# Acly/dlimgedit

Measured on AMD Instinct MI355X. Metric: images/sec encode+mask @1024x1024, higher is better.
Workload: dtype f16; 1 GPU; SAM vit_b encoder + 1 point prompt, 1 image(s)/GPU/step, 1024x1024 RGBA, inputs and masks resident in HBM; timed through the extension entry point dlimg_amd_encode_and_mask (device pointers in and out) -- the drop-in table itself, host buffers in and out, is `abi_path`; weights=seeded synthetic, lanes_per_gpu=4, lanes_fed_by_the_step_queue=3, requests_coalesced_per_pass=4, passes_queued_per_lane=2

## Files before the change

### dlimgedit_amd/csrc/kernels/decoder.hip

```cpp
#include "device_common.hpp"
#include "kernels.hpp"

#include <cstring>
#include <mutex>
#include <type_traits>

namespace dlimg {
namespace {

#include "gemm_f16_tile.inc"

constexpr int OUT_TOK = 5;
constexpr int DIM = 256;
constexpr int INNER = 128;
constexpr int HEADS = 8;
constexpr int NTOK_IMG = 4096;

template <int TOK, typename Prompts>
DLIMG_DEVICE void prompt_token_column(const Prompts& pr, int p, int c, const float* __restrict__ gauss,
                                      const float* __restrict__ point_embed, const float* __restrict__ not_a_point,
                                      const float* __restrict__ iou_token, const float* __restrict__ mask_tokens,
                                      float (&out)[TOK]) {
    constexpr int NPTS = TOK - OUT_TOK;
    out[0] = iou_token[c];
// ... 493 lines not shown
}

template <int TOK>
constexpr size_t TML_LDS = (size_t)(INNER * DIM + TL_ROW_SLICE<TOK> * INNER + TL_ROW_SLICE<TOK> * DIM) * 4 + 2 * TL_ROW_SLICE<TOK> * 8;
template <int TOK, int NR, int COLS>
DLIMG_DEVICE void token_merge_linear_body(const float* __restrict__ part, const k::TokenLinear& out,
                                          const float* __restrict__ out_wt, const k::TokenLinear& next, int p0, float* lds) {
    float* wt = lds;
    float* att = wt + INNER * DIM;
    float* y = att + TL_ROW_SLICE<TOK> * INNER;
    float2_t* stat_res = reinterpret_cast<float2_t*>(y + TL_ROW_SLICE<TOK> * DIM);
    float2_t* stat_in = stat_res + TL_ROW_SLICE<TOK>;
    const int row0 = p0 * TOK, row1 = row0 + NR;
    const int first = blockIdx.x * COLS;
    const int c = threadIdx.x, lane = lane_id(), wave = c >> 6;
    for (int k = wave; k < INNER; k += 4) glds16(out_wt + (size_t)k * DIM + lane * 4, wt + k * DIM);
    TokenColumn col = token_column_prefetch(next, first, row0, row1);
    float res[NR];
#pragma unroll
    for (int r = 0; r < NR; ++r) res[r] = out.resid.x ? out.resid.x[(size_t)(row0 + r) * DIM + c] : 0.f;
    const bool res_ln = out.resid.x && out.resid.ln_w;
    const float rw = res_ln ? out.resid.ln_w[c] : 1.f, rb = res_ln ? out.resid.ln_b[c] : 0.f;
    const float ob = out.b ? out.b[c] : 0.f;
    const float nw = next.in.ln_w ? next.in.ln_w[c] : 1.f, nb = next.in.ln_w ? next.in.ln_b[c] : 0.f;
    float nadd[NR];
#pragma unroll
    for (int r = 0; r < NR; ++r) nadd[r] = next.in.add ? next.in.add[(size_t)(row0 + r) * DIM + c] : 0.f;
    merge_partials<TOK, NR>(part, p0, 0, att);
    if (res_ln) token_row_stats(out.resid, row1, stat_res - row0, row0);
    asm volatile("s_waitcnt vmcnt(0)" ::: "memory");
    __syncthreads();
    float acc[NR];
#pragma unroll
    for (int r = 0; r < NR; ++r) acc[r] = 0.f;
#pragma unroll 2
    for (int k4 = 0; k4 < INNER / 4; ++k4) {
        float w[4];
        float4_t a[NR];
#pragma unroll
        for (int i = 0; i < 4; ++i) w[i] = wt[(4 * k4 + i) * DIM + c];
#pragma unroll
        for (int r = 0; r < NR; ++r) a[r] = reinterpret_cast<const float4_t*>(att)[r * (INNER / 4) + k4];
#pragma unroll
        for (int r = 0; r < NR; ++r)
#pragma unroll
            for (int i = 0; i < 4; ++i) acc[r] = fmaf(a[r][i], w[i], acc[r]);
    }
#pragma unroll
    for (int r = 0; r < NR; ++r) {
        float v = acc[r] + ob;
        if (out.resid.x) v += res_ln ? (res[r] - stat_res[r][0]) * stat_res[r][1] * rw + rb : res[r];
        y[r * DIM + c] = v;
        if (blockIdx.x == 0) out.Y[(size_t)(row0 + r) * DIM + c] = v;
    }
    __syncthreads();
    if (next.in.ln_w) {
        lds_row_stats(y, NR, next.in.eps, stat_in);
        __syncthreads();
    }
    if (next.in.ln_w || next.in.add) {
#pragma unroll
        for (int r = 0; r < NR; ++r) {
            float v = y[r * DIM + c];
            if (next.in.ln_w) v = (v - stat_in[r][0]) * stat_in[r][1] * nw + nb;
            y[r * DIM + c] = v + nadd[r];
        }
        __syncthreads();
    }
#pragma unroll 1
    for (int i = 0; i < COLS / 4; ++i) {
        const TokenColumn following = token_column_prefetch(next, first + 4 * min(i + 1, COLS / 4 - 1), row0, row1);
        token_linear_columns<TOK, NR>(next, first + 4 * i, y, nullptr, nullptr, col, row0);
        col = following;
    }
}
template <int TOK, int COLS>
__global__ __launch_bounds__(256) void token_merge_linear_kernel(const float* __restrict__ part, k::TokenLinear out,
                                                                 const float* __restrict__ out_wt, k::TokenLinear next, int P) {
    extern __shared__ __attribute__((aligned(16))) float lds[];
    token_merge_linear_body<TOK, TOK, COLS>(part, out, out_wt, next, blockIdx.y, lds);
}

constexpr int HEAD_THREADS = 1024;
static_assert(DIM == 64 * 4, "one float4 of the weight row per lane");

template <int N_OUT>
DLIMG_DEVICE void head_layer(const float* x , const float* __restrict__ w, const float* __restrict__ b, int n_out,
                             bool relu, float* y) {
    constexpr int WAVES = HEAD_THREADS / 64, ROWS = (N_OUT + WAVES - 1) / WAVES;
    const int lane = lane_id(), wave = threadIdx.x >> 6;
    const float4_t v = reinterpret_cast<const float4_t*>(x)[lane];
    float4_t wr[ROWS];
#pragma unroll
    for (int r = 0; r < ROWS; ++r) {
        const int n = wave + r * WAVES;
        wr[r] = float4_t{0.f, 0.f, 0.f, 0.f};
        if (n < n_out) wr[r] = reinterpret_cast<const float4_t*>(w + (size_t)n * DIM)[lane];
    }
#pragma unroll
    for (int r = 0; r < ROWS; ++r) {
        const int n = wave + r * WAVES;
        const float acc = wave_sum((v[0] * wr[r][0] + v[1] * wr[r][1]) + (v[2] * wr[r][2] + v[3] * wr[r][3]));
        if (lane == 0 && n < n_out) {
            const float out = acc + b[n];
            y[n] = relu ? fmaxf(out, 0.f) : out;
        }
    }
}

template <int TOK >
__global__ __launch_bounds__(HEAD_THREADS) void output_heads_kernel(const float* __restrict__ part, k::TokenLinear out,
                                                                    const float* __restrict__ out_wt, k::TokenRows norm,
                                                                    k::HeadWeights hw, float* __restrict__ hyper,
                                                                    float* __restrict__ iou) {
    __shared__ __attribute__((aligned(16))) float x0[DIM], x1[DIM], x2[DIM], att[INNER];
    __shared__ float opart[4][DIM];
    __shared__ float2_t stat[1], stat_res[1];
    const int p = blockIdx.x, mi = blockIdx.y;
    const int tok = mi < 4 ? 1 + mi : 0;
    const int row = p * TOK + tok;
    const int c = threadIdx.x & (DIM - 1), kq = threadIdx.x >> 8;
    float w[INNER / 4];
#pragma unroll
    for (int k = 0; k < INNER / 4; ++k) w[k] = out_wt[(size_t)(kq * (INNER / 4) + k) * DIM + c];
    float res = 0.f, rw = 1.f, rb = 0.f;
    if (out.resid.x && kq == 0) {
        res = out.resid.x[(size_t)row * DIM + c];
        if (out.resid.ln_w) { rw = out.resid.ln_w[c]; rb = out.resid.ln_b[c]; }
    }
    const float ob = (out.b && kq == 0) ? out.b[c] : 0.f;
    if (threadIdx.x < INNER) merge_partials_one(part, p, tok, TOK, att);
    if (out.resid.x && out.resid.ln_w && (threadIdx.x >> 6) == 15) {
        const int lane = lane_id();
        const float4_t v = reinterpret_cast<const float4_t*>(out.resid.x + (size_t)row * DIM)[lane];
        const float mean = wave_sum((v[0] + v[1]) + (v[2] + v[3])) * (1.0f / DIM);
        const float4_t d = v - mean;
        const float var = wave_sum((d[0] * d[0] + d[1] * d[1]) + (d[2] * d[2] + d[3] * d[3])) * (1.0f / DIM);
        if (lane == 0) stat_res[0] = float2_t{mean, 1.0f / sqrtf(var + out.resid.eps)};
    }
    __syncthreads();
    {
        float acc = 0.f;
#pragma unroll
        for (int k = 0; k < INNER / 4; ++k) acc = fmaf(att[kq * (INNER / 4) + k], w[k], acc);
        opart[kq][c] = acc;
    }
    __syncthreads();
    if (kq == 0) {
        float v = ((opart[0][c] + opart[1][c]) + (opart[2][c] + opart[3][c])) + ob;
        if (out.resid.x) v += out.resid.ln_w ? (res - stat_res[0][0]) * stat_res[0][1] * rw + rb : res;
        x1[c] = v;
    }
    __syncthreads();
    if (threadIdx.x < 64) lds_row_stats(x1, 1, norm.eps, stat);
    __syncthreads();
    if (threadIdx.x < DIM)
        x0[threadIdx.x] = (x1[threadIdx.x] - stat[0][0]) * stat[0][1] * norm.ln_w[threadIdx.x] + norm.ln_b[threadIdx.x];
    __syncthreads();
    head_layer<DIM>(x0, hw.w[mi][0], hw.b[mi][0], DIM, true, x1);
    __syncthreads();
    head_layer<DIM>(x1, hw.w[mi][1], hw.b[mi][1], DIM, true, x2);
    __syncthreads();
    float* dst = mi < 4 ? hyper + ((size_t)p * 4 + mi) * 32 : iou + (size_t)p * 4;
    head_layer<32>(x2, hw.w[mi][2], hw.b[mi][2], mi < 4 ? 32 : 4, false, dst);
}

template <int TOK>
struct StartPrompts {
    static constexpr int NPTS = TOK - OUT_TOK;
    float coords[k::kDecoderMaxPrompts * NPTS * 2];
    float labels[k::kDecoderMaxPrompts * NPTS];
    const float* emb[k::kDecoderMaxPrompts];
};
template <int TOK>
struct DecoderStart {
    StartPrompts<TOK> prompts;
    const float* gauss; const float* point_embed; const float* not_a_point; const float* iou_token; const float* mask_tokens;
    float* tokens;
    LinJob first;
    int lin_blocks, lin_cols;
    const float* no_mask; float* keys; half_t* keys_h; size_t n4_per_prompt; int P;
};
template <int TOK>
__global__ __launch_bounds__(256) void decoder_start_kernel(DecoderStart<TOK> a) {
    __shared__ __attribute__((aligned(16))) float rows[TL_ROW_SLICE<TOK> * DIM];
    const int c = threadIdx.x;
    if ((int)blockIdx.x < a.P) {
        float v[TOK];
        prompt_token_column<TOK>(a.prompts, blockIdx.x, c, a.gauss, a.point_embed, a.not_a_point, a.iou_token, a.mask_tokens, v);
#pragma unroll
        for (int t = 0; t < TOK; ++t) a.tokens[((size_t)blockIdx.x * TOK + t) * DIM + c] = v[t];
        return;
    }
    if ((int)blockIdx.x < a.P + a.lin_blocks) {
        const int bid = blockIdx.x - a.P;
        int o = 0, first = (bid % a.lin_cols) * 4;
        while (o + 1 < a.first.count && first >= a.first.op[o].N) { first -= a.first.op[o].N; ++o; }
        const k::TokenLinear& op = a.first.op[o];
        const int row0 = (bid / a.lin_cols) * TL_ROW_SLICE<TOK>, row1 = min(a.first.rows, row0 + TL_ROW_SLICE<TOK>);
        const TokenColumn w_first = token_column_prefetch(op, first, row0, row1);
        for (int p = row0 / TOK; p * TOK < row1; ++p) {
            float v[TOK];
            prompt_token_column<TOK>(a.prompts, p, c, a.gauss, a.point_embed, a.not_a_point, a.iou_token, a.mask_tokens, v);
#pragma unroll
            for (int t = 0; t < TOK; ++t) rows[(p * TOK + t - row0) * DIM + c] = v[t];
        }
        __syncthreads();
        DLIMG_FOR_SLICE_ROWS(row1 - row0, token_linear_columns<TOK, NR>(op, first, rows, nullptr, nullptr, w_first, row0);)
        return;
    }
    const float* __restrict__ no_mask = a.no_mask;
    float* __restrict__ keys = a.keys;
    half_t* __restrict__ keys_h = a.keys_h;
    const size_t n4_per_prompt = a.n4_per_prompt;
    const int P = a.P, skip = a.P + a.lin_blocks;
    const size_t total = n4_per_prompt * P;
    const size_t nblk = gridDim.x - skip;
    for (size_t i = (blockIdx.x - skip) * (size_t)blockDim.x + threadIdx.x; i < total; i += nblk * blockDim.x) {
        const size_t p = i / n4_per_prompt, j = i % n4_per_prompt;
        float4_t v = reinterpret_cast<const float4_t*>(a.prompts.emb[p])[j];
        v += reinterpret_cast<const float4_t*>(no_mask)[j % (DIM / 4)];
        reinterpret_cast<float4_t*>(keys)[i] = v;
        reinterpret_cast<half4_t*>(keys_h)[i] = half4_t{(half_t)v[0], (half_t)v[1], (half_t)v[2], (half_t)v[3]};
    }
}

}

#define DLIMG_FOR_TOKENS(T, who, ...)                                        \
    if ((T) == 7) { constexpr int TOK = 7; __VA_ARGS__ }                     \
    else if ((T) == 8) { constexpr int TOK = 8; __VA_ARGS__ }                \
    else { throw_error(who ": 7 or 8 tokens per prompt"); }

namespace k {

void decoder_start(const DecoderPrompts& prompts, const float* gauss, const float* point_embed, const float* not_a_point,
                   const float* iou_token, const float* mask_tokens, float* tokens, const TokenLinear* first, int n_first,
                   const float* no_mask, float* keys, half_t* keys_h, int P, int T, hipStream_t s) {
    if (P <= 0) return;
    if (!decoder_tokens_supported(T)) throw_error("decoder_start: 7 or 8 tokens per prompt");
    if (P > decoder_max_prompts(T) || n_first < 0 || n_first > TL_MAX_OPS) throw_error("decoder_start: too many prompts or layers");
    const size_t n4 = (size_t)NTOK_IMG * DIM / 4;
    const size_t total = n4 * P;
    const int key_blocks = (int)((total + 255) / 256 > 4096 ? 4096 : (total + 255) / 256);
    int cols = 0;
    for (int i = 0; i < n_first; ++i) {
        if (first[i].K != DIM || first[i].N <= 0 || first[i].N % 4 || first[i].in.ln_w || first[i].in.add || first[i].resid.x)
// ... 129 lines not shown
```

### dlimgedit_amd/csrc/kernels/elementwise.hip

```cpp
#include "device_common.hpp"
#include "kernels.hpp"

namespace dlimg {
namespace {


__constant__ float c_mean[3] = {123.675f, 116.28f, 103.53f};
__constant__ float c_std[3] = {58.395f, 57.12f, 57.375f};

struct ChannelMap { int bytes; int idx[3]; };

__host__ __device__ inline ChannelMap channel_map(int channels) {
    switch (channels) {
    case 1: return {1, {0, 0, 0}};
    case 3: return {3, {0, 1, 2}};
    case 5: return {4, {2, 1, 0}};
    case 6: return {4, {1, 2, 3}};
    default: return {4, {0, 1, 2}};
    }
}

constexpr int PRE_MAX_JOBS = 16;
struct PreJob { const uint8_t* img; half_t* out; int w, h, stride, channels; };
struct PreJobs { PreJob j[PRE_MAX_JOBS]; };

__global__ __launch_bounds__(256) void preprocess_kernel(PreJobs jobs) {
    const PreJob job = jobs.j[blockIdx.y];
    const uint8_t* __restrict__ img = job.img;
    half_t* __restrict__ out = job.out;
    const int w = job.w, h = job.h, stride = job.stride, channels = job.channels;
    const int lane = lane_id();
    const int pair = blockIdx.x * 4 + (threadIdx.x >> 6);
    const int iy = lane >> 2, p = (lane >> 1) & 1, half = lane & 1;
    const int patch = pair * 2 + p;
    const int py = patch >> 6, px = patch & 63;
    const int y = py * 16 + iy;
    const int x0 = px * 16 + half * 8;
    const ChannelMap cm = channel_map(channels);

    float v[3][8];
#pragma unroll
    for (int c = 0; c < 3; ++c)
#pragma unroll
        for (int i = 0; i < 8; ++i) v[c][i] = 0.f;

    if (y < h && x0 < w) {
        const uint8_t* row = img + (size_t)y * stride;
        const bool fast = cm.bytes == 4 && x0 + 8 <= w && ((((uintptr_t)row) + (size_t)x0 * 4) & 15) == 0;
        if (fast) {
            const uint4* src = reinterpret_cast<const uint4*>(row + (size_t)x0 * 4);
            uint4 q0 = src[0], q1 = src[1];
            uint32_t px32[8] = {q0.x, q0.y, q0.z, q0.w, q1.x, q1.y, q1.z, q1.w};
#pragma unroll
            for (int i = 0; i < 8; ++i)
#pragma unroll
                for (int c = 0; c < 3; ++c) {
                    float u = (float)((px32[i] >> (8 * cm.idx[c])) & 0xffu);
                    v[c][i] = (u - c_mean[c]) / c_std[c];
                }
        } else {
#pragma unroll
            for (int i = 0; i < 8; ++i) {
                if (x0 + i < w) {
                    const uint8_t* px8 = row + (size_t)(x0 + i) * cm.bytes;
#pragma unroll
                    for (int c = 0; c < 3; ++c) v[c][i] = ((float)px8[cm.idx[c]] - c_mean[c]) / c_std[c];
                }
            }
        }
    }
    half_t* dst = out + (size_t)patch * 768 + iy * 16 + half * 8;
#pragma unroll
    for (int c = 0; c < 3; ++c) {
        half8_t o;
#pragma unroll
        for (int i = 0; i < 8; ++i) o[i] = (half_t)v[c][i];
        store16_result(dst + c * 256, o);
    }
}

constexpr int LN_MAX_PER_LANE = 20;

template <int ACT>
__global__ __launch_bounds__(256) void layernorm_kernel(const float* __restrict__ x, const float* __restrict__ w,
                                                        const float* __restrict__ b, float eps, int rows, int D,
                                                        float* out_f32, half_t* out_h) {
    const int row = blockIdx.x * 4 + (threadIdx.x >> 6);
    if (row >= rows) return;
    const int lane = lane_id();
    const float* xr = x + (size_t)row * D;
    float v[LN_MAX_PER_LANE];
    float s = 0.f;
#pragma unroll
    for (int i = 0; i < LN_MAX_PER_LANE; ++i) {
        int c = i * 64 + lane;
        v[i] = c < D ? xr[c] : 0.f;
        s += v[i];
    }
    const float mean = wave_sum(s) / (float)D;
    float q = 0.f;
#pragma unroll
    for (int i = 0; i < LN_MAX_PER_LANE; ++i) {
        int c = i * 64 + lane;
        float d = c < D ? v[i] - mean : 0.f;
        v[i] = d;
        q += d * d;
    }
    const float rstd = 1.0f / sqrtf(wave_sum(q) / (float)D + eps);
#pragma unroll
    for (int i = 0; i < LN_MAX_PER_LANE; ++i) {
        int c = i * 64 + lane;
        if (c < D) {
            float y = v[i] * rstd * w[c] + b[c];
            if (ACT == k::ACT_GELU) y = gelu_erf(y);
            if (out_f32) out_f32[(size_t)row * D + c] = y;
            if (out_h) out_h[(size_t)row * D + c] = (half_t)y;
        }
    }
}

constexpr int LN_MAX_VEC = 5;
template <int ACT>
__global__ __launch_bounds__(256) void layernorm_vec_kernel(const float* __restrict__ x, const float* __restrict__ w,
                                                            const float* __restrict__ b, float eps, int rows, int D,
                                                            float* out_f32, half_t* out_h, int* nonfinite) {
    const int row = blockIdx.x * 4 + (threadIdx.x >> 6);
    if (row >= rows) return;
    const int lane = lane_id();
    const int nv = D >> 8;
    const float4_t* xr = reinterpret_cast<const float4_t*>(x + (size_t)row * D);
    float4_t v[LN_MAX_VEC];
    float s = 0.f;
#pragma unroll
    for (int i = 0; i < LN_MAX_VEC; ++i) {
        v[i] = float4_t{0.f, 0.f, 0.f, 0.f};
        if (i < nv) v[i] = xr[i * 64 + lane];
        s += (v[i][0] + v[i][1]) + (v[i][2] + v[i][3]);
    }
    const float mean = wave_sum(s) / (float)D;
    float q = 0.f;
#pragma unroll
    for (int i = 0; i < LN_MAX_VEC; ++i) {
        if (i < nv) {
            v[i] -= mean;
            q += (v[i][0] * v[i][0] + v[i][1] * v[i][1]) + (v[i][2] * v[i][2] + v[i][3] * v[i][3]);
        }
    }
    const float rstd = 1.0f / sqrtf(wave_sum(q) / (float)D + eps);
    if (nonfinite && lane == 0 && !(fabsf(mean) < INFINITY && fabsf(rstd) < INFINITY)) *nonfinite = 1;
#pragma unroll
    for (int i = 0; i < LN_MAX_VEC; ++i) {
        if (i < nv) {
            const int c4 = i * 64 + lane;
            const float4_t ww = reinterpret_cast<const float4_t*>(w)[c4], bb = reinterpret_cast<const float4_t*>(b)[c4];
            float4_t y = v[i] * rstd * ww + bb;
            if (ACT == k::ACT_GELU) {
#pragma unroll
                for (int e = 0; e < 4; ++e) y[e] = gelu_erf(y[e]);
            }
            if (out_f32) store16_result(out_f32 + (size_t)row * D + (size_t)c4 * 4, y);
            if (out_h) {
                half4_t h = {(half_t)y[0], (half_t)y[1], (half_t)y[2], (half_t)y[3]};
                reinterpret_cast<half4_t*>(out_h + (size_t)row * D)[c4] = h;
            }
        }
    }
}

__global__ __launch_bounds__(256) void add_cast_kernel(const float* __restrict__ a, const float* __restrict__ b,
                                                       size_t b_mod, size_t n4, float* out_f32, half_t* out_h) {
    for (size_t i = blockIdx.x * (size_t)blockDim.x + threadIdx.x; i < n4; i += (size_t)gridDim.x * blockDim.x) {
        float4_t v = reinterpret_cast<const float4_t*>(a)[i];
        if (b) {
            float4_t u = *reinterpret_cast<const float4_t*>(b + (i * 4) % b_mod);
            v += u;
        }
        if (out_f32) store16_result(out_f32 + i * 4, v);
        if (out_h) {
            half4_t o = {(half_t)v[0], (half_t)v[1], (half_t)v[2], (half_t)v[3]};
            reinterpret_cast<half4_t*>(out_h)[i] = o;
        }
    }
}

__global__ __launch_bounds__(256) void cast_f16_kernel(const float* __restrict__ in, half_t* __restrict__ out, size_t n) {
    for (size_t i = blockIdx.x * (size_t)blockDim.x + threadIdx.x; i < n; i += (size_t)gridDim.x * blockDim.x)
        out[i] = (half_t)in[i];
}

__global__ __launch_bounds__(256) void im2col3x3_kernel(const half_t* __restrict__ in, int B, int C,
                                                        half_t* __restrict__ out) {
    const int cpr = C / 8;
    const size_t total = (size_t)B * 4096 * 9 * cpr;
    for (size_t i = blockIdx.x * (size_t)blockDim.x + threadIdx.x; i < total; i += (size_t)gridDim.x * blockDim.x) {
        int ch = (int)(i % cpr);
        size_t t = i / cpr;
        int tap = (int)(t % 9);
        size_t tok = t / 9;
        int b = (int)(tok >> 12), y = (int)((tok >> 6) & 63), x = (int)(tok & 63);
        int yy = y + tap / 3 - 1, xx = x + tap % 3 - 1;
        half8_t v = zero_h8();
        if (yy >= 0 && yy < 64 && xx >= 0 && xx < 64)
            v = *reinterpret_cast<const half8_t*>(in + (((size_t)b * 4096 + yy * 64 + xx) * C) + ch * 8);
        store16_result(out + (tok * 9 + tap) * C + ch * 8, v);
    }
}

inline int grid_for(size_t work_items, int cap = 2048) {
    size_t g = (work_items + 255) / 256;
    return (int)(g < 1 ? 1 : (g > (size_t)cap ? cap : g));
}

}

namespace k {

void preprocess_batch(const PreImage* images, int count, hipStream_t s) {
    for (int base = 0; base < count; base += PRE_MAX_JOBS) {
        const int n = count - base < PRE_MAX_JOBS ? count - base : PRE_MAX_JOBS;
        PreJobs jobs{};
        for (int i = 0; i < n; ++i) {
            const PreImage& im = images[base + i];
            if (!im.img || !im.patches) throw_error("preprocess: null buffer");
            if (im.w <= 0 || im.h <= 0 || im.w > 1024 || im.h > 1024) throw_error("preprocess: image must be 1..1024 pixels per side");
            const int bytes = im.channels > 4 ? 4 : im.channels;
            if (!(im.channels == 1 || im.channels == 3 || im.channels == 4 || im.channels == 5 || im.channels == 6))
                throw_error("preprocess: unsupported channel order");
            if (im.stride < im.w * bytes) throw_error("preprocess: stride smaller than one row of pixels");
            jobs.j[i] = PreJob{im.img, im.patches, im.w, im.h, im.stride, im.channels};
        }
        hipLaunchKernelGGL(preprocess_kernel, dim3(512, n), dim3(256), 0, s, jobs);
    }
}

void preprocess(const uint8_t* img, int w, int h, int stride, int channels, half_t* patches, hipStream_t s) {
    const PreImage one{img, w, h, stride, channels, patches};
    preprocess_batch(&one, 1, s);
}

void layernorm(const float* x, const float* w, const float* b, float eps, int rows, int D, int act, float* out_f32,
               half_t* out_h, hipStream_t s, int* nonfinite) {
    if (rows <= 0) return;
    if (D <= 0 || D > LN_MAX_PER_LANE * 64) throw_error("layernorm: row length must be in 1..1280");
    dim3 grid((rows + 3) / 4);
    const bool aligned = !(((uintptr_t)x | (uintptr_t)w | (uintptr_t)b | (uintptr_t)out_f32) & 15) && !((uintptr_t)out_h & 7);
    if (D % 256 == 0 && aligned) {
        if (act == ACT_GELU)
            hipLaunchKernelGGL(layernorm_vec_kernel<ACT_GELU>, grid, dim3(256), 0, s, x, w, b, eps, rows, D, out_f32, out_h, nonfinite);
        else
            hipLaunchKernelGGL(layernorm_vec_kernel<ACT_NONE>, grid, dim3(256), 0, s, x, w, b, eps, rows, D, out_f32, out_h, nonfinite);
        return;
    }
    if (nonfinite) throw_error("layernorm: the non-finite report needs rows that are a multiple of 256 long");
    if (act == ACT_GELU)
        hipLaunchKernelGGL(layernorm_kernel<ACT_GELU>, grid, dim3(256), 0, s, x, w, b, eps, rows, D, out_f32, out_h);
    else
        hipLaunchKernelGGL(layernorm_kernel<ACT_NONE>, grid, dim3(256), 0, s, x, w, b, eps, rows, D, out_f32, out_h);
}

void add_cast(const float* a, const float* b, size_t b_mod, size_t n, float* out_f32, half_t* out_h, hipStream_t s) {
    if (n == 0) return;
    if (n % 4 || (b && (b_mod % 4 || b_mod == 0))) throw_error("add_cast: lengths must be multiples of 4");
    hipLaunchKernelGGL(add_cast_kernel, dim3(grid_for(n / 4)), dim3(256), 0, s, a, b, b_mod, n / 4, out_f32, out_h);
}

void cast_f16(const float* in, half_t* out, size_t n, hipStream_t s) {
    if (n == 0) return;
    hipLaunchKernelGGL(cast_f16_kernel, dim3(grid_for(n)), dim3(256), 0, s, in, out, n);
}

void im2col3x3(const half_t* in, int B, int C, half_t* out, hipStream_t s) {
    if (B <= 0 || C <= 0 || C % 8) throw_error("im2col3x3: channel count must be a positive multiple of 8");
    hipLaunchKernelGGL(im2col3x3_kernel, dim3(grid_for((size_t)B * 4096 * 9 * (C / 8))), dim3(256), 0, s, in, B, C, out);
}

}
}
```

### dlimgedit_amd/csrc/kernels/kernels.hpp

```cpp
#pragma once

#include <hip/hip_runtime.h>
#include <stdint.h>

namespace dlimg {

typedef _Float16 half_t;

[[noreturn]] void throw_error(const char* msg);

namespace k {

class LdsOptIn {
  public:
    static constexpr int kMaxDevices = 64;
    void ensure(const void* kernel, size_t bytes, const char* refused_message) {
        int dev = 0;
        if (hipGetDevice(&dev) != hipSuccess || dev < 0 || dev >= kMaxDevices) throw_error("kernel launch: no current HIP device");
        int st = __atomic_load_n(&state_[dev], __ATOMIC_ACQUIRE);
        if (st == 0) {
            st = hipFuncSetAttribute(kernel, hipFuncAttributeMaxDynamicSharedMemorySize, (int)bytes) == hipSuccess ? 1 : -1;
            if (st < 0) (void)hipGetLastError();
            __atomic_store_n(&state_[dev], st, __ATOMIC_RELEASE);
        }
        if (st < 0) throw_error(refused_message);
    }

  private:
    int state_[kMaxDevices] = {};
};

enum Act { ACT_NONE = 0, ACT_GELU = 1 };

struct GemmArgs {
    const half_t* A = nullptr;  int lda = 0;
    const half_t* W = nullptr;  int ldw = 0;
    const float* bias = nullptr;
    const float* resid = nullptr; int ldr = 0; int resid_mod = 1;
    float* out_f32 = nullptr;   int ldc32 = 0;
    half_t* out_h = nullptr;    int ldc16 = 0;
    const half_t* resid_h = nullptr; const half_t* resid_l = nullptr; int ldrs = 0;
    half_t* out_l = nullptr;
    int M = 0, N = 0, K = 0;
    int act = ACT_NONE;
    float* stats_out = nullptr;
    const float* ln_stats = nullptr;
    int ln_groups = 0;
    const float* ln_colsum = nullptr;
    float ln_eps = 0.f;
    bool shared_gpu = false;
    bool alone = false;
    int tile = -1;
    int unit_rows = 0;
    unsigned long long* stamps = nullptr;
};
const char* gemm_check(const GemmArgs&);
bool gemm_tile_fits(const GemmArgs&, int tile);
int gemm_choose_tile(GemmArgs&);
void gemm(const GemmArgs&, hipStream_t, hipEvent_t start = nullptr, hipEvent_t stop = nullptr);

void layernorm(const float* x, const float* w, const float* b, float eps, int rows, int D, int act,
               float* out_f32, half_t* out_h, hipStream_t, int* nonfinite = nullptr);

void preprocess(const uint8_t* img, int w, int h, int stride, int channels, half_t* patches, hipStream_t);
struct PreImage { const uint8_t* img; int w, h, stride, channels; half_t* patches; };
void preprocess_batch(const PreImage* images, int count, hipStream_t);

struct ResizeAxis { const int* first; const int* count; const float* coef; int taps; int out; };
void resize_srgb(const uint8_t* src, int w, int h, int stride, int C, const ResizeAxis& ax, const ResizeAxis& ay,
                 const float* decode_lut, const uint32_t* encode_tab, float* tmp, uint8_t* dst, hipStream_t);

void add_cast(const float* a, const float* b, size_t b_mod, size_t n, float* out_f32, half_t* out_h, hipStream_t);
void im2col3x3(const half_t* in, int B, int C, half_t* out, hipStream_t);
void cast_f16(const float* in, half_t* out, size_t n, hipStream_t);

void attention_window(const half_t* qkv, const half_t* qkv_pad, const half_t* rel_h, const half_t* rel_w,
                      half_t* out, int B, int heads, int hd, hipStream_t);
float attention_global_q_scale(int hd);
float attention_global_rel_scale(int hd);
void attention_global(const half_t* qkv, const half_t* rel_h, const half_t* rel_w, half_t* out, int B,
                      int heads, int hd, hipStream_t);

constexpr int kDecoderMaxRows = 112;
constexpr bool decoder_tokens_supported(int T) { return T == 7 || T == 8; }
constexpr int decoder_max_prompts(int T) { return kDecoderMaxRows / T; }
size_t token_to_image_scratch_floats(int P, int T);
struct TokenRows {
    const float* x = nullptr;
    const float* ln_w = nullptr;
    const float* ln_b = nullptr;
    float eps = 0.f;
    const float* add = nullptr;
};
struct TokenLinear {
    TokenRows in;
    int K = 0;
    const float* W = nullptr;
    const float* b = nullptr;
    TokenRows resid;
    float* Y = nullptr;
    int N = 0;
    int relu = 0;
};
constexpr int kDecoderMaxPrompts = 16;
constexpr int kDecoderMaxPoints = 3;
struct DecoderPrompts {
    float coords[kDecoderMaxPrompts * kDecoderMaxPoints * 2];
    float labels[kDecoderMaxPrompts * kDecoderMaxPoints];
    const float* emb[kDecoderMaxPrompts];
};
void decoder_start(const DecoderPrompts& prompts, const float* gauss, const float* point_embed, const float* not_a_point,
                   const float* iou_token, const float* mask_tokens, float* tokens, const TokenLinear* first, int n_first,
                   const float* no_mask, float* keys, half_t* keys_h, int P, int T, hipStream_t s);
void token_linears(const TokenLinear* ops, int count, int rows, int T, hipStream_t);
void token_self_attention_out(const float* q, const float* k, const float* v, const TokenLinear& out, int P, int T, hipStream_t);
bool token_self_attention_out_with_gemm(const float* q, const float* k, const float* v, const TokenLinear& out, int P, int T,
                                        const GemmArgs& g, hipStream_t);
void token_to_image_partials(const float* q, const TokenLinear* q_proj, const half_t* K, int ldk, const half_t* V, int ldv,
                             float* scratch, int P, int T, hipStream_t);
void token_merge_linear(const float* scratch, const TokenLinear& out, const float* out_wt, const TokenLinear& next, int P,
                        int T, hipStream_t);
void image_update(const half_t* q, int ldq, const float* tk, const float* tv, const half_t* W, const float* bias,
                  const float* ln_w, const float* ln_b, float eps, float* keys, half_t* keys_h, int P, int T, hipStream_t);
void upscale_logits(const half_t* keys_h, const half_t* W1, const float* b1, const float* ln_w, const float* ln_b, float eps,
                    const half_t* W2, const float* b2, const float* hyper, float* logits, int P, hipStream_t);
struct HeadWeights { const float* w[5][3]; const float* b[5][3]; };
void output_heads(const float* scratch, const TokenLinear& out, const float* out_wt, const TokenRows& norm ,
                  const HeadWeights& hw, float* hyper , float* iou , int P, int T, hipStream_t);

void birefnet_prepare_image(const uint8_t* pixels, int w, int h, int stride, int bytes_pp, const float mean[3],
                            const float std[3], float* out, hipStream_t s);
void birefnet_process_mask(const float* logits, int w, int h, uint8_t* out, hipStream_t s);

struct PostJob { const float* src; const float* select_iou; uint8_t* dst; int out_w, out_h, pre_w, pre_h; };
void postprocess_masks(const PostJob* jobs_host, int count, hipStream_t);

}
}
```

### dlimgedit_amd/csrc/sam_model.cpp

```cpp
#include "sam_model.hpp"
#include "image_memory.hpp"
#include "mask_pieces.hpp"

#include <algorithm>
#include <cmath>
#include <cstdlib>
#include <chrono>
#include <cstring>

namespace dlimg {

namespace {

constexpr float kLnEps = 1e-6f;
constexpr float kDecLnEps = 1e-5f;

struct Loader {
    WeightFile const& file;
    hipStream_t stream;
    DeviceBuffer<float> staging;

    void f32(std::string const& name, std::vector<int64_t> const& dims, DeviceBuffer<float>& dst) {
        HostTensor const& t = file.get(name, dims);
        dst.reserve(t.numel());
// ... 686 lines not shown
    };
    auto reads_stream = [&](k::GemmArgs& a, LinearH const& lin, NormW const& norm) {
        if (fused) {
            a.ln_stats = xstat_.get(); a.ln_groups = stat_groups; a.ln_colsum = lin.colsum.get(); a.ln_eps = kLnEps;
        } else {
            timed(ST_LAYERNORM, (double)M * D * 6, [&] {
                k::layernorm(x_.get(), norm.w.get(), norm.b.get(), kLnEps, M, D, k::ACT_NONE, nullptr, xn_.get(), stream_);
            });
        }
        a.A = xn_.get(); a.lda = D; a.W = lin.w.get(); a.ldw = D; a.bias = lin.b.get(); a.M = M; a.N = lin.out; a.K = D;
    };

    k::GemmArgs g;
    g.A = patches_.get(); g.lda = kPatchK; g.W = W.patch_.w.get(); g.ldw = kPatchK; g.bias = W.patch_.b.get();
    g.resid = W.pos_embed_.get(); g.ldr = D; g.resid_mod = kTokens; g.K = kPatchK;
    writes_stream(g);
    gemm(g, ST_GEMM_PATCH);

    for (EncoderLayer const& L : W.layers_) {
        g = k::GemmArgs{};
        reads_stream(g, L.qkv, L.ln1);
        g.out_h = qkv_.get(); g.ldc16 = 3 * D;
        gemm(g);
        if (L.global) {
            const double fl = (double)batch * (4.0 * kTokens * (double)kTokens * D + 4.0 * kTokens * 64.0 * hd * H);
            timed(ST_ATTN_GLOBAL, fl, [&] {
                k::attention_global(qkv_.get(), L.rel_h16.get(), L.rel_w16.get(), att_.get(), batch, H, hd, stream_);
            });
        } else {
            const double fl = (double)batch * 25.0 * (4.0 * 196.0 * 196.0 * D + 4.0 * 196.0 * 14.0 * hd * H);
            timed(ST_ATTN_WINDOW, fl, [&] {
                k::attention_window(qkv_.get(), L.qkv_pad.get(), L.rel_h16.get(), L.rel_w16.get(), att_.get(), batch, H, hd,
                                    stream_);
            });
        }
        g = k::GemmArgs{};
        g.A = att_.get(); g.lda = D; g.W = L.proj.w.get(); g.ldw = D; g.bias = L.proj.b.get(); g.K = D;
        stream_residual(g);
        writes_stream(g);
        gemm(g, ST_GEMM_PROJ);
        g = k::GemmArgs{};
        reads_stream(g, L.fc1, L.ln2);
        g.act = k::ACT_GELU; g.out_h = hid_.get(); g.ldc16 = mlp;
        gemm(g);
        g = k::GemmArgs{};
        g.A = hid_.get(); g.lda = mlp; g.W = L.fc2.w.get(); g.ldw = mlp; g.bias = L.fc2.b.get(); g.K = mlp;
        stream_residual(g);
        writes_stream(g);
        gemm(g, ST_GEMM_FC2);
    }

    if (!fused) {
        timed(ST_ENC_OTHER, (double)M * D * 6, [&] {
            k::add_cast(x_.get(), nullptr, 0, (size_t)M * D, nullptr, xn_.get(), stream_);
        });
    }
    g = k::GemmArgs{};
    g.A = xn_.get(); g.lda = D; g.W = W.neck1_.w.get(); g.ldw = D;
    g.out_f32 = neck_f32_.get(); g.ldc32 = kEmbedDim; g.M = M; g.N = kEmbedDim; g.K = D;
    gemm(g);
    timed(ST_LAYERNORM, (double)M * kEmbedDim * 6, [&] {
        k::layernorm(neck_f32_.get(), W.neck_ln1_.w.get(), W.neck_ln1_.b.get(), kLnEps, M, kEmbedDim, k::ACT_NONE, nullptr,
                     att_.get(), stream_);
    });
    timed(ST_ENC_OTHER, (double)M * kEmbedDim * 2 * 10, [&] {
        k::im2col3x3(att_.get(), batch, kEmbedDim, hid_.get(), stream_);
    });
    g = k::GemmArgs{};
    g.A = hid_.get(); g.lda = 9 * kEmbedDim; g.W = W.neck2_.w.get(); g.ldw = 9 * kEmbedDim;
    g.out_f32 = neck_f32_.get(); g.ldc32 = kEmbedDim; g.M = M; g.N = kEmbedDim; g.K = 9 * kEmbedDim;
    gemm(g);
    float* direct = (emb_dst && batch == 1 && emb_dst[0]) ? emb_dst[0] : nullptr;
    if (!pass_flags_) {
        HIP_CHECK(hipHostMalloc(reinterpret_cast<void**>(&pass_flags_), kPassFlags * sizeof(int), hipHostMallocDefault));
        std::memset(pass_flags_, 0, kPassFlags * sizeof(int));
    }
    const unsigned flag_slot = pass_counter_++ % kPassFlags;
    if (flag_owner_[flag_slot]) {
        flag_owner_[flag_slot]->settle();
        flag_owner_[flag_slot].reset();
    }
    pass_flag_ = pass_flags_ + flag_slot;
    *pass_flag_ = 0;
    timed(ST_LAYERNORM, (double)M * kEmbedDim * 8, [&] {
        k::layernorm(neck_f32_.get(), W.neck_ln2_.w.get(), W.neck_ln2_.b.get(), kLnEps, M, kEmbedDim, k::ACT_NONE,
                     direct ? direct : emb_.get(), nullptr, stream_, pass_flag_);
    });
    if (emb_dst && !direct) {
        const size_t n = (size_t)kTokens * kEmbedDim;
        for (int i = 0; i < batch; ++i)
            if (emb_dst[i])
                HIP_CHECK(hipMemcpyAsync(emb_dst[i], emb_.get() + i * n, n * sizeof(float), hipMemcpyDeviceToDevice, stream_));
    }
    HIP_CHECK(hipGetLastError());
    mark_activity();
}


void SamModel::reserve_decoder(int count) {
    if (count <= dec_count_) return;
    HIP_CHECK(hipStreamSynchronize(stream_));
    const size_t P = count, M = P * kTokens;
    keys_.reserve(M * 256);
    keys_h_.reserve(M * 256);
    kqv_h_.reserve(M * 384);
    logits_.reserve(P * 4 * kLowRes * kLowRes);
    iou_.reserve(P * 4);
    hyper_.reserve(P * 4 * 32);
    const size_t T = P * kDecMaxTokens;
    tokens_.reserve(T * 256);
    queries_.reserve(T * 256);
    tk_.reserve(T * 256);
    tv_.reserve(T * 256);
    sq_.reserve(T * 256);
    sk_.reserve(T * 256);
    sv_.reserve(T * 256);
    tsa_.reserve(T * 256);
    tt2i_.reserve(T * 256);
    t2i_part_.reserve(k::token_to_image_scratch_floats((int)P, kDecMaxTokens));
    tmlp_.reserve(T * 2048);
    dec_count_ = count;
}

void SamModel::decode(float const* const* emb, float const* coords, float const* labels, int count, int points) {
    DLIMG_ASSERT(count > 0);
    DLIMG_ASSERT(points >= 2 && points <= k::kDecoderMaxPoints);
    static_assert(5 + k::kDecoderMaxPoints == kDecMaxTokens && k::decoder_tokens_supported(kDecTokens) &&
                  k::decoder_tokens_supported(kDecMaxTokens), "the kernels are built for these token counts");
    reserve_decoder(count);
    const int chunk = k::decoder_max_prompts(5 + points);
    for (int c0 = 0; c0 < count; c0 += chunk)
        decode_chunk(emb + c0, coords + (size_t)c0 * points * 2, labels + (size_t)c0 * points, std::min(chunk, count - c0), c0,
                     points);
    mark_activity();
}

void SamModel::decode_chunk(float const* const* emb, float const* coords, float const* labels, int count, int first,
                            int points) {
    SamWeights const& W = *weights_;
    const int TOK = 5 + points;
    const int P = count, M = P * kTokens, T = P * TOK;
    hipStream_t s = stream_;
    float* logits_out = logits_.get() + (size_t)first * 4 * kLowRes * kLowRes;
    float* iou_out = iou_.get() + (size_t)first * 4;

    auto body = [&] {
        k::DecoderPrompts prompts{};
        std::memcpy(prompts.coords, coords, (size_t)P * points * 2 * sizeof(float));
        std::memcpy(prompts.labels, labels, (size_t)P * points * sizeof(float));
        for (int i = 0; i < P; ++i) prompts.emb[i] = emb[i];

        float const* qpe = tokens_.get();
        k::TokenRows cur;
        auto rows_of = [&](k::TokenRows r, bool with_pe) { if (with_pe) r.add = qpe; return r; };
        auto lin = [&](k::TokenRows in, int K, LinearF const& l, k::TokenRows resid, float* Y, int relu) {
            k::TokenLinear op;
            op.in = in; op.K = K; op.W = l.w.get(); op.b = l.b.get(); op.resid = resid; op.Y = Y; op.N = l.out; op.relu = relu;
            return op;
        };
        auto plain = [&](float const* x) { k::TokenRows r; r.x = x; return r; };
        auto normed = [&](float const* x, NormW const& n) {
            k::TokenRows r; r.x = x; r.ln_w = n.w.get(); r.ln_b = n.b.get(); r.eps = kDecLnEps; return r;
        };
        auto img_gemm_args = [&](LinearH const& l, DeviceBuffer<float> const& pos) {
            k::GemmArgs g;
            g.A = keys_h_.get(); g.lda = 256; g.W = l.w.get(); g.ldw = 256; g.bias = l.b.get();
            g.resid = pos.get(); g.ldr = l.out; g.resid_mod = kTokens;
            g.out_h = kqv_h_.get(); g.ldc16 = l.out; g.M = M; g.N = l.out; g.K = 256;
            g.shared_gpu = shared_gpu_;
            g.unit_rows = kTokens;
            return g;
// ... 293 lines not shown
```

Before: 908.1 images/s.

## Prefetch head weights early in output heads and scatter neck layernorm to destinations

The output-heads kernel now issues its MLP weight-row loads and biases ahead of the preceding barriers, splitting each layer's rows into an early batch and a late batch. This hides global-memory latency behind the attention projection and layernorm phases. Biases are held one per lane and broadcast with a shuffle instead of a per-row load. Separately, the neck layernorm can write each image's rows directly into its per-request embedding buffer, removing the device-to-device copies when batches coalesce requests. Both add register pressure and code complexity.

```diff
diff --git a/dlimgedit_amd/csrc/kernels/decoder.hip b/dlimgedit_amd/csrc/kernels/decoder.hip
--- a/dlimgedit_amd/csrc/kernels/decoder.hip
+++ b/dlimgedit_amd/csrc/kernels/decoder.hip
@@ -599,27 +599,39 @@
 }
 
 constexpr int HEAD_THREADS = 1024;
+constexpr int HEAD_WAVES = HEAD_THREADS / 64;
+constexpr int HEAD_ROWS = DIM / HEAD_WAVES;
+constexpr int HEAD_EARLY1 = 12;
+constexpr int HEAD_EARLY2 = 8;
 static_assert(DIM == 64 * 4, "one float4 of the weight row per lane");
-
-template <int N_OUT>
-DLIMG_DEVICE void head_layer(const float* x , const float* __restrict__ w, const float* __restrict__ b, int n_out,
-                             bool relu, float* y) {
-    constexpr int WAVES = HEAD_THREADS / 64, ROWS = (N_OUT + WAVES - 1) / WAVES;
+static_assert(HEAD_ROWS * HEAD_WAVES == DIM && HEAD_ROWS <= 64, "lane r of a wave carries the bias of the wave's row r");
+
+template <int NR>
+DLIMG_DEVICE void head_rows_request(const float* __restrict__ w, int n_out, int r0, float4_t (&wr)[NR]) {
+    const int lane = lane_id(), wave = threadIdx.x >> 6;
+#pragma unroll
+    for (int r = 0; r < NR; ++r) {
+        const int n = wave + (r0 + r) * HEAD_WAVES;
+        wr[r] = float4_t{0.f, 0.f, 0.f, 0.f};
+        if (n < n_out) wr[r] = reinterpret_cast<const float4_t*>(w + (size_t)n * DIM)[lane];
+    }
+}
+DLIMG_DEVICE float head_bias_request(const float* __restrict__ b, int n_out) {
+    const int lane = lane_id(), n = (threadIdx.x >> 6) + lane * HEAD_WAVES;
+    return (lane < HEAD_ROWS && n < n_out) ? b[n] : 0.f;
+}
+template <int NR>
+DLIMG_DEVICE void head_rows_apply(const float* x , const float4_t (&wr)[NR], float bias, int n_out, int r0, bool relu,
+                                  float* y) {
     const int lane = lane_id(), wave = threadIdx.x >> 6;
     const float4_t v = reinterpret_cast<const float4_t*>(x)[lane];
-    float4_t wr[ROWS];
-#pragma unroll
-    for (int r = 0; r < ROWS; ++r) {
-        const int n = wave + r * WAVES;
-        wr[r] = float4_t{0.f, 0.f, 0.f, 0.f};
-        if (n < n_out) wr[r] = reinterpret_cast<const float4_t*>(w + (size_t)n * DIM)[lane];
-    }
-#pragma unroll
-    for (int r = 0; r < ROWS; ++r) {
-        const int n = wave + r * WAVES;
+#pragma unroll
+    for (int r = 0; r < NR; ++r) {
+        const int n = wave + (r0 + r) * HEAD_WAVES;
         const float acc = wave_sum((v[0] * wr[r][0] + v[1] * wr[r][1]) + (v[2] * wr[r][2] + v[3] * wr[r][3]));
+        const float bn = __shfl(bias, r0 + r, 64);
         if (lane == 0 && n < n_out) {
-            const float out = acc + b[n];
+            const float out = acc + bn;
             y[n] = relu ? fmaxf(out, 0.f) : out;
         }
     }
@@ -636,6 +648,7 @@
     const int p = blockIdx.x, mi = blockIdx.y;
     const int tok = mi < 4 ? 1 + mi : 0;
     const int row = p * TOK + tok;
+    const int n_last = mi < 4 ? 32 : 4;
     const int c = threadIdx.x & (DIM - 1), kq = threadIdx.x >> 8;
     float w[INNER / 4];
 #pragma unroll
@@ -655,6 +668,11 @@
         const float var = wave_sum((d[0] * d[0] + d[1] * d[1]) + (d[2] * d[2] + d[3] * d[3])) * (1.0f / DIM);
         if (lane == 0) stat_res[0] = float2_t{mean, 1.0f / sqrtf(var + out.resid.eps)};
     }
+    float4_t w1a[HEAD_EARLY1], w1b[HEAD_ROWS - HEAD_EARLY1], w3[32 / HEAD_WAVES];
+    head_rows_request<HEAD_EARLY1>(hw.w[mi][0], DIM, 0, w1a);
+    const float b1 = head_bias_request(hw.b[mi][0], DIM), b2 = head_bias_request(hw.b[mi][1], DIM),
+                b3 = head_bias_request(hw.b[mi][2], n_last);
+    const float fw = kq == 0 ? norm.ln_w[c] : 0.f, fb = kq == 0 ? norm.ln_b[c] : 0.f;
     __syncthreads();
     {
         float acc = 0.f;
@@ -662,6 +680,9 @@
         for (int k = 0; k < INNER / 4; ++k) acc = fmaf(att[kq * (INNER / 4) + k], w[k], acc);
         opart[kq][c] = acc;
     }
+    float4_t w2a[HEAD_EARLY2], w2b[HEAD_ROWS - HEAD_EARLY2];
+    head_rows_request<HEAD_ROWS - HEAD_EARLY1>(hw.w[mi][0], DIM, HEAD_EARLY1, w1b);
+    head_rows_request<HEAD_EARLY2>(hw.w[mi][1], DIM, 0, w2a);
     __syncthreads();
     if (kq == 0) {
         float v = ((opart[0][c] + opart[1][c]) + (opart[2][c] + opart[3][c])) + ob;
@@ -671,15 +692,18 @@
     __syncthreads();
     if (threadIdx.x < 64) lds_row_stats(x1, 1, norm.eps, stat);
     __syncthreads();
-    if (threadIdx.x < DIM)
-        x0[threadIdx.x] = (x1[threadIdx.x] - stat[0][0]) * stat[0][1] * norm.ln_w[threadIdx.x] + norm.ln_b[threadIdx.x];
-    __syncthreads();
-    head_layer<DIM>(x0, hw.w[mi][0], hw.b[mi][0], DIM, true, x1);
-    __syncthreads();
-    head_layer<DIM>(x1, hw.w[mi][1], hw.b[mi][1], DIM, true, x2);
+    if (threadIdx.x < DIM) x0[threadIdx.x] = (x1[threadIdx.x] - stat[0][0]) * stat[0][1] * fw + fb;
+    __syncthreads();
+    head_rows_apply<HEAD_EARLY1>(x0, w1a, b1, DIM, 0, true, x1);
+    head_rows_apply<HEAD_ROWS - HEAD_EARLY1>(x0, w1b, b1, DIM, HEAD_EARLY1, true, x1);
+    head_rows_request<HEAD_ROWS - HEAD_EARLY2>(hw.w[mi][1], DIM, HEAD_EARLY2, w2b);
+    head_rows_request<32 / HEAD_WAVES>(hw.w[mi][2], n_last, 0, w3);
+    __syncthreads();
+    head_rows_apply<HEAD_EARLY2>(x1, w2a, b2, DIM, 0, true, x2);
+    head_rows_apply<HEAD_ROWS - HEAD_EARLY2>(x1, w2b, b2, DIM, HEAD_EARLY2, true, x2);
     __syncthreads();
     float* dst = mi < 4 ? hyper + ((size_t)p * 4 + mi) * 32 : iou + (size_t)p * 4;
-    head_layer<32>(x2, hw.w[mi][2], hw.b[mi][2], mi < 4 ? 32 : 4, false, dst);
+    head_rows_apply<32 / HEAD_WAVES>(x2, w3, b3, n_last, 0, false, dst);
 }
 
 template <int TOK>
diff --git a/dlimgedit_amd/csrc/kernels/elementwise.hip b/dlimgedit_amd/csrc/kernels/elementwise.hip
--- a/dlimgedit_amd/csrc/kernels/elementwise.hip
+++ b/dlimgedit_amd/csrc/kernels/elementwise.hip
@@ -1,5 +1,7 @@
 #include "device_common.hpp"
 #include "kernels.hpp"
+
+#include <type_traits>
 
 namespace dlimg {
 namespace {
@@ -120,10 +122,12 @@
 }
 
 constexpr int LN_MAX_VEC = 5;
-template <int ACT>
+struct NoUnits {};
+template <int ACT, bool UNITS = false>
 __global__ __launch_bounds__(256) void layernorm_vec_kernel(const float* __restrict__ x, const float* __restrict__ w,
                                                             const float* __restrict__ b, float eps, int rows, int D,
-                                                            float* out_f32, half_t* out_h, int* nonfinite) {
+                                                            float* out_f32, half_t* out_h, int* nonfinite,
+                                                            std::conditional_t<UNITS, k::LayernormUnits, NoUnits> units) {
     const int row = blockIdx.x * 4 + (threadIdx.x >> 6);
     if (row >= rows) return;
     const int lane = lane_id();
@@ -158,7 +162,12 @@
 #pragma unroll
                 for (int e = 0; e < 4; ++e) y[e] = gelu_erf(y[e]);
             }
-            if (out_f32) store16_result(out_f32 + (size_t)row * D + (size_t)c4 * 4, y);
+            if constexpr (UNITS) {
+                const int u = row / units.rows_per_unit;
+                store16_result(units.dst[u] + (size_t)(row - u * units.rows_per_unit) * D + (size_t)c4 * 4, y);
+            } else if (out_f32) {
+                store16_result(out_f32 + (size_t)row * D + (size_t)c4 * 4, y);
+            }
             if (out_h) {
                 half4_t h = {(half_t)y[0], (half_t)y[1], (half_t)y[2], (half_t)y[3]};
                 reinterpret_cast<half4_t*>(out_h + (size_t)row * D)[c4] = h;
@@ -246,9 +255,9 @@
     const bool aligned = !(((uintptr_t)x | (uintptr_t)w | (uintptr_t)b | (uintptr_t)out_f32) & 15) && !((uintptr_t)out_h & 7);
     if (D % 256 == 0 && aligned) {
         if (act == ACT_GELU)
-            hipLaunchKernelGGL(layernorm_vec_kernel<ACT_GELU>, grid, dim3(256), 0, s, x, w, b, eps, rows, D, out_f32, out_h, nonfinite);
+            hipLaunchKernelGGL(layernorm_vec_kernel<ACT_GELU>, grid, dim3(256), 0, s, x, w, b, eps, rows, D, out_f32, out_h, nonfinite, NoUnits{});
         else
-            hipLaunchKernelGGL(layernorm_vec_kernel<ACT_NONE>, grid, dim3(256), 0, s, x, w, b, eps, rows, D, out_f32, out_h, nonfinite);
+            hipLaunchKernelGGL(layernorm_vec_kernel<ACT_NONE>, grid, dim3(256), 0, s, x, w, b, eps, rows, D, out_f32, out_h, nonfinite, NoUnits{});
         return;
     }
     if (nonfinite) throw_error("layernorm: the non-finite report needs rows that are a multiple of 256 long");
@@ -258,6 +267,22 @@
         hipLaunchKernelGGL(layernorm_kernel<ACT_NONE>, grid, dim3(256), 0, s, x, w, b, eps, rows, D, out_f32, out_h);
 }
 
+void layernorm_units(const float* x, const float* w, const float* b, float eps, int rows, int D, const LayernormUnits& units,
+                     hipStream_t s, int* nonfinite) {
+    if (rows <= 0) return;
+    if (D <= 0 || D % 256 || D > LN_MAX_VEC * 256) throw_error("layernorm_units: row length must be a multiple of 256 up to 1280");
+    if (units.rows_per_unit <= 0 || rows % units.rows_per_unit || rows / units.rows_per_unit > kLayernormMaxUnits)
+        throw_error("layernorm_units: whole units of rows, at most 16 of them");
+    uintptr_t bits = (uintptr_t)x | (uintptr_t)w | (uintptr_t)b;
+    for (int u = 0; u < rows / units.rows_per_unit; ++u) {
+        if (!units.dst[u]) throw_error("layernorm_units: every unit needs a destination");
+        bits |= (uintptr_t)units.dst[u];
+    }
+    if (bits & 15) throw_error("layernorm_units: operands must be 16-byte aligned");
+    hipLaunchKernelGGL((layernorm_vec_kernel<ACT_NONE, true>), dim3((rows + 3) / 4), dim3(256), 0, s, x, w, b, eps, rows, D,
+                       (float*)nullptr, (half_t*)nullptr, nonfinite, units);
+}
+
 void add_cast(const float* a, const float* b, size_t b_mod, size_t n, float* out_f32, half_t* out_h, hipStream_t s) {
     if (n == 0) return;
     if (n % 4 || (b && (b_mod % 4 || b_mod == 0))) throw_error("add_cast: lengths must be multiples of 4");
diff --git a/dlimgedit_amd/csrc/kernels/kernels.hpp b/dlimgedit_amd/csrc/kernels/kernels.hpp
--- a/dlimgedit_amd/csrc/kernels/kernels.hpp
+++ b/dlimgedit_amd/csrc/kernels/kernels.hpp
@@ -61,6 +61,10 @@
 
 void layernorm(const float* x, const float* w, const float* b, float eps, int rows, int D, int act,
                float* out_f32, half_t* out_h, hipStream_t, int* nonfinite = nullptr);
+constexpr int kLayernormMaxUnits = 16;
+struct LayernormUnits { float* dst[kLayernormMaxUnits]; int rows_per_unit; };
+void layernorm_units(const float* x, const float* w, const float* b, float eps, int rows, int D, const LayernormUnits& units,
+                     hipStream_t, int* nonfinite = nullptr);
 
 void preprocess(const uint8_t* img, int w, int h, int stride, int channels, half_t* patches, hipStream_t);
 struct PreImage { const uint8_t* img; int w, h, stride, channels; half_t* patches; };
diff --git a/dlimgedit_amd/csrc/sam_model.cpp b/dlimgedit_amd/csrc/sam_model.cpp
--- a/dlimgedit_amd/csrc/sam_model.cpp
+++ b/dlimgedit_amd/csrc/sam_model.cpp
@@ -792,11 +792,21 @@
     }
     pass_flag_ = pass_flags_ + flag_slot;
     *pass_flag_ = 0;
+    bool scatter = emb_dst && !direct && batch <= k::kLayernormMaxUnits;
+    for (int i = 0; scatter && i < batch; ++i) scatter = emb_dst[i] != nullptr;
     timed(ST_LAYERNORM, (double)M * kEmbedDim * 8, [&] {
-        k::layernorm(neck_f32_.get(), W.neck_ln2_.w.get(), W.neck_ln2_.b.get(), kLnEps, M, kEmbedDim, k::ACT_NONE,
-                     direct ? direct : emb_.get(), nullptr, stream_, pass_flag_);
+        if (scatter) {
+            k::LayernormUnits units{};
+            for (int i = 0; i < batch; ++i) units.dst[i] = emb_dst[i];
+            units.rows_per_unit = kTokens;
+            k::layernorm_units(neck_f32_.get(), W.neck_ln2_.w.get(), W.neck_ln2_.b.get(), kLnEps, M, kEmbedDim, units, stream_,
+                               pass_flag_);
+        } else {
+            k::layernorm(neck_f32_.get(), W.neck_ln2_.w.get(), W.neck_ln2_.b.get(), kLnEps, M, kEmbedDim, k::ACT_NONE,
+                         direct ? direct : emb_.get(), nullptr, stream_, pass_flag_);
+        }
     });
-    if (emb_dst && !direct) {
+    if (emb_dst && !direct && !scatter) {
         const size_t n = (size_t)kTokens * kEmbedDim;
         for (int i = 0; i < batch; ++i)
             if (emb_dst[i])
```

Measured after the change: 908.2 images/s (median of 4 runs). About the same (+0.0%).
